# PRBonn/SHINE_mapping

Measured on AMD Instinct MI355X. Metric: trained SDF samples/sec (fwd+bwd), higher is better.
Workload: dtype f32; 1 GPU; maicity (BASELINE config 2): MaiCity-like 100 m street map, batch mode, 262144 points/iter/GPU, 4-level octree, F=8, decoder 8-32-32-1, BCE, f32; 100 poses x 64 beams x 1800 azimuths; points_per_iter_per_gpu=262144, levels=4, pool_samples=65450694, feature_table_bytes=14510624, parallelism=dp1

## Files before the change

include/shine_hip.h:

```cpp
#ifndef SHINE_HIP_H_
#define SHINE_HIP_H_

#include <stddef.h>
#include <stdint.h>

#ifdef __cplusplus
extern "C" {
#endif

#define SHINE_MAX_LEVELS 8
#define SHINE_FEATURE_DIM 8
#define SHINE_HIDDEN_DIM 32
#define SHINE_MLP_PARAMS 1377

#define SHINE_OK 0
#define SHINE_E_INVALID (-1)
#define SHINE_E_HIP (-2)
#define SHINE_E_NOMEM (-3)
#define SHINE_E_STATE (-4)

typedef struct shine_tables shine_tables;

#define SHINE_SURF_PARTS 64
typedef struct shine_next_draw {
  int64_t pool_size, n;
  uint64_t seed;
  uint64_t* stream_state;
  int32_t* idx_out;
  const uint32_t* surf_bits;
  int64_t* surf_parts;
  void* workspace;
} shine_next_draw;

typedef struct shine_draw_rider {
  int64_t pool_size, n;
  uint64_t seed;
  uint64_t* state;
  int32_t parity;
  double* block_sum[2];
  int32_t* idx_out;
  const uint32_t* surf_bits;
  int64_t* surf_parts[2];
  float* zero_ptr;
  int64_t zero_bytes;
} shine_draw_rider;
int shine_draw_rider_prime(const shine_draw_rider* r, uint64_t first_stream_id, void* stream);

typedef struct shine_reg_rider {
  const float* last[SHINE_MAX_LEVELS];
  const float* imp[SHINE_MAX_LEVELS];
  uint32_t* stamp[SHINE_MAX_LEVELS];
  uint32_t epoch;
  float* acc;
} shine_reg_rider;

typedef struct shine_step_config {
  int32_t n_levels;
  int32_t max_level;
  int32_t poly_int_on;
  int32_t reduction_sum;
  int32_t eikonal_on;
  int32_t decoder_grad_on;
  int32_t sorted_input;
  int32_t kernel_variant;
  float sigma;
  float weight_e;
  double inv_n;
  int64_t n_global;
  int32_t sort_origin[3];
  int32_t sort_bits[3];
  int32_t loss_weight_on;
  int64_t* adam_state;
  float adam_beta1, adam_beta2;
  double* zero_f64;
  int32_t n_surf_parts;
  const shine_next_draw* next_draw;
  int32_t defer_reduce;
// ... 259 lines not shown
```

shine_mapping_amd/_lib.py:

```python
import ctypes as C
import os

_HERE = os.path.dirname(os.path.abspath(__file__))
LIB_PATH = os.path.join(_HERE, "lib", "libshine_hip.so")
CHECK_LIB_PATH = os.path.join(_HERE, "lib", "libshine_check.so")

MAX_LEVELS = 8
FEATURE_DIM = 8
HIDDEN_DIM = 32
MLP_PARAMS = 1377


class NextDraw(C.Structure):
    _fields_ = [("pool_size", C.c_int64), ("n", C.c_int64), ("seed", C.c_uint64), ("stream_state", C.c_void_p),
                ("idx_out", C.c_void_p), ("surf_bits", C.c_void_p), ("surf_parts", C.c_void_p), ("workspace", C.c_void_p)]


class RegRider(C.Structure):

    _fields_ = [("last", C.c_void_p * 8), ("imp", C.c_void_p * 8), ("stamp", C.c_void_p * 8), ("epoch", C.c_uint32),
                ("acc", C.c_void_p)]


class DrawRider(C.Structure):

    _fields_ = [("pool_size", C.c_int64), ("n", C.c_int64), ("seed", C.c_uint64), ("state", C.c_void_p), ("parity", C.c_int32),
                ("block_sum", C.c_void_p * 2), ("idx_out", C.c_void_p), ("surf_bits", C.c_void_p), ("surf_parts", C.c_void_p * 2),
                ("zero_ptr", C.c_void_p), ("zero_bytes", C.c_int64)]


class StepConfig(C.Structure):

    _fields_ = [
        ("n_levels", C.c_int32),
        ("max_level", C.c_int32),
        ("poly_int_on", C.c_int32),
        ("reduction_sum", C.c_int32),
        ("eikonal_on", C.c_int32),
        ("decoder_grad_on", C.c_int32),
        ("sorted_input", C.c_int32),
        ("kernel_variant", C.c_int32),
        ("sigma", C.c_float),
        ("weight_e", C.c_float),
        ("inv_n", C.c_double),
        ("n_global", C.c_int64),
        ("sort_origin", C.c_int32 * 3),
        ("sort_bits", C.c_int32 * 3),
        ("loss_weight_on", C.c_int32),
        ("adam_state", C.c_void_p),
        ("adam_beta1", C.c_float),
        ("adam_beta2", C.c_float),
        ("zero_f64", C.c_void_p),
        ("n_surf_parts", C.c_int32),
        ("next_draw", C.POINTER(NextDraw)),
        ("defer_reduce", C.c_int32),
        ("reg_rider", C.POINTER(RegRider)),
        ("draw_rider", C.POINTER(DrawRider)),
    ]


_P = C.c_void_p
# ... 248 lines not shown
```

shine_mapping_amd/csrc/shine_graph.hip:

```cpp
#include <cstdlib>
#include <vector>

#include "shine_finish_args.hpp"
#include "shine_tile16.hpp"

struct shine_iter_graph {
  int unroll = 0;
  hipGraph_t graph = nullptr;
  hipGraphExec_t exec = nullptr;
  std::vector<hipGraphNode_t> step_nodes, fin_nodes;
  shine::StepLaunch step = {};
  shine::FinLaunch fin = {};
  bool have_step = false, have_fin = false, dirty = false;
  const void* built_step_fn = nullptr;
  const void* built_fin_fn = nullptr;
  long long commits = 0, builds = 0;
  hipEvent_t last_replay = nullptr;
  bool replayed = false;
  float* image = nullptr;
};

namespace shine {

static void graph_drop(shine_iter_graph* g) {
  if (g->exec) (void)hipGraphExecDestroy(g->exec);
  if (g->graph) (void)hipGraphDestroy(g->graph);
  g->exec = nullptr;
  g->graph = nullptr;
  g->step_nodes.clear();
  g->fin_nodes.clear();
}

static hipKernelNodeParams step_params(shine_iter_graph* g, void** kp) {
  hipKernelNodeParams p = {};
  kp[0] = &g->step.a;
  p.func = const_cast<void*>(g->step.fn);
  p.gridDim = g->step.grid;
  p.blockDim = g->step.block;
  p.sharedMemBytes = 0;
  p.kernelParams = kp;
  p.extra = nullptr;
  return p;
}

static hipKernelNodeParams fin_params(shine_iter_graph* g, void** kp) {
  hipKernelNodeParams p = {};
  kp[0] = &g->fin.a;
  kp[1] = &g->fin.fb;
  kp[2] = &g->fin.db;
  p.func = const_cast<void*>(g->fin.fn);
  p.gridDim = g->fin.grid;
  p.blockDim = g->fin.block;
  p.sharedMemBytes = 0;
  p.kernelParams = kp;
  p.extra = nullptr;
  return p;
}

static int graph_build(shine_iter_graph* g) {
  graph_drop(g);
  SHINE_HIP_CHECK(hipGraphCreate(&g->graph, 0));
  void* skp[1];
  void* fkp[3];
  hipKernelNodeParams sp = step_params(g, skp), fp = fin_params(g, fkp);
  hipGraphNode_t prev = nullptr;
  for (int u = 0; u < g->unroll; ++u) {
    hipGraphNode_t sn = nullptr, fn = nullptr;
    SHINE_HIP_CHECK(hipGraphAddKernelNode(&sn, g->graph, prev ? &prev : nullptr, prev ? 1 : 0, &sp));
    SHINE_HIP_CHECK(hipGraphAddKernelNode(&fn, g->graph, &sn, 1, &fp));
    g->step_nodes.push_back(sn);
    g->fin_nodes.push_back(fn);
    prev = fn;
  }
  SHINE_HIP_CHECK(hipGraphInstantiate(&g->exec, g->graph, nullptr, nullptr, 0));
  g->built_step_fn = g->step.fn;
  g->built_fin_fn = g->fin.fn;
  ++g->builds;
  return SHINE_OK;
}

}

using namespace shine;

extern "C" int shine_iter_graph_create(int32_t unroll, shine_iter_graph** out) {
  if (!out || unroll < 1 || unroll > 256) return set_error(SHINE_E_INVALID, "shine_iter_graph_create: 1 <= unroll <= 256");
  shine_iter_graph* g = new (std::nothrow) shine_iter_graph();
  if (!g) return set_error(SHINE_E_NOMEM, "shine_iter_graph_create: out of host memory");
  g->unroll = unroll;
  *out = g;
  return SHINE_OK;
}

extern "C" int shine_iter_graph_destroy(shine_iter_graph* g) {
  if (!g) return SHINE_OK;
// ... 43 lines not shown
                                           const int64_t* n_surf, double* loss_parts, const float* const* feats_last,
                                           const float* const* importance, unsigned char* const* touched,
                                           const int32_t* grad_on, float lambda_forget, double* reg_out, int32_t n_tensors,
                                           float* const* params, float* const* grads, float* const* exp_avg,
                                           float* const* exp_avg_sq, const int64_t* numel, const float* lr_dev,
                                           const int32_t* lr_index, const float* weight_decay, float beta1, float beta2,
                                           float eps, const int64_t* step_state, const shine_next_draw* next_draw,
                                           int32_t active_rows) {
  if (!g) return set_error(SHINE_E_INVALID, "shine_iter_graph_set_finish: null graph");
  FinLaunch fl;
  int rc = prepare_finish(&fl, cfg, n, workspace, n_surf, loss_parts, feats_last, importance, touched, grad_on, lambda_forget,
                          reg_out, n_tensors, params, grads, exp_avg, exp_avg_sq, numel, lr_dev, lr_index, weight_decay, beta1,
                          beta2, eps, step_state, next_draw, active_rows);
  if (rc != SHINE_OK) return rc;
  g->fin = fl;
  g->have_fin = true;
  g->dirty = true;
  return SHINE_OK;
}

extern "C" int shine_iter_graph_commit(shine_iter_graph* g) {
  if (!g || !g->have_step || !g->have_fin)
    return set_error(SHINE_E_STATE, "shine_iter_graph_commit: set_step and set_finish first");
  if (g->fin.a.partials != g->step.a.partials || g->fin.a.nblocks != g->step.blocks)
    return set_error(SHINE_E_INVALID, "shine_iter_graph_commit: the tail must consume the step's workspace (same buffer, same batch size)");
  g->fin.a.op_image = g->step.a.op_image ? g->image : nullptr;
  ++g->commits;
  g->dirty = false;
  if (g->replayed) {
    SHINE_HIP_CHECK(hipEventSynchronize(g->last_replay));
    g->replayed = false;
  }
  if (g->exec && g->built_step_fn == g->step.fn && g->built_fin_fn == g->fin.fn) {
    void* skp[1];
    void* fkp[3];
    hipKernelNodeParams sp = step_params(g, skp), fp = fin_params(g, fkp);
    bool ok = true;
    for (int u = 0; u < g->unroll && ok; ++u) {
      ok = hipGraphExecKernelNodeSetParams(g->exec, g->step_nodes[u], &sp) == hipSuccess &&
           hipGraphExecKernelNodeSetParams(g->exec, g->fin_nodes[u], &fp) == hipSuccess;
    }
    if (ok) return SHINE_OK;
    (void)hipGetLastError();
  }
  return graph_build(g);
}

extern "C" int shine_iter_graph_launch(shine_iter_graph* g, int32_t replays, void* stream) {
  if (!g || !g->exec || g->dirty) return set_error(SHINE_E_STATE, "shine_iter_graph_launch: commit first");
  if (replays < 1) return SHINE_OK;
  if (!g->last_replay) SHINE_HIP_CHECK(hipEventCreateWithFlags(&g->last_replay, hipEventDisableTiming));
  if (g->step.a.op_image) {
    const int rc = launch_operand_image(g->step.a, g->image, (hipStream_t)stream);
    if (rc != SHINE_OK) return rc;
  }
  for (int r = 0; r < replays; ++r) SHINE_HIP_CHECK(hipGraphLaunch(g->exec, (hipStream_t)stream));
  SHINE_HIP_CHECK(hipEventRecord(g->last_replay, (hipStream_t)stream));
  g->replayed = true;
  return SHINE_OK;
}

extern "C" int shine_iter_graph_stats(const shine_iter_graph* g, int64_t* commits, int64_t* builds) {
  if (!g) return set_error(SHINE_E_INVALID, "shine_iter_graph_stats: null graph");
  if (commits) *commits = g->commits;
  if (builds) *builds = g->builds;
  return SHINE_OK;
}
// ... 1 lines not shown
```

shine_mapping_amd/csrc/shine_step_common.hpp:

```cpp
#pragma once
#include "shine_internal.hpp"

namespace shine {

constexpr int LCAP = 4;

constexpr int PART_TRASH = SHINE_MLP_PARAMS;
constexpr int PART_FLOATS = PART_TRASH + SHINE_MAX_LEVELS * 8;
constexpr int PART_LOSS = 1444;
constexpr int PART_STRIDE = 1456;

struct V1Level {
  const unsigned long long* keys;
  const int4* vals;
  const float* feat;
  float* grad;
  unsigned int shift, mask;
  float res;
  int pad;
};

struct V1Args {
  V1Level lv[LCAP];
  long long rows[LCAP];
// ... 58 lines not shown
  const int cx = (c >> 2) & 1, cy = (c >> 1) & 1, cz = c & 1;
  const float px = cx ? X.t : 1.0f - X.t, py = cy ? Y.t : 1.0f - Y.t, pz = cz ? Z.t : 1.0f - Z.t;
  const float gx = cx ? X.dt : -X.dt, gy = cy ? Y.dt : -Y.dt, gz = cz ? Z.dt : -Z.dt;
  out[0] = gx * py * pz;
  out[1] = px * gy * pz;
  out[2] = px * py * gz;
}

typedef float f32x2_t __attribute__((ext_vector_type(2)));
__device__ __forceinline__ void corner_dw_pair(const Axis& X, const Axis& Y, const Axis& Z, int cp, f32x2_t out[3]) {
  const int cx = (cp >> 1) & 1, cy = cp & 1;
  const float px = cx ? X.t : 1.0f - X.t, py = cy ? Y.t : 1.0f - Y.t;
  const float gx = cx ? X.dt : -X.dt, gy = cy ? Y.dt : -Y.dt;
  const f32x2_t pz = {1.0f - Z.t, Z.t}, gz = {-Z.dt, Z.dt};
  const float a = gx * py, b = px * gy, c = px * py;
  out[0] = (f32x2_t){a, a} * pz;
  out[1] = (f32x2_t){b, b} * pz;
  out[2] = (f32x2_t){c, c} * gz;
}

__device__ __forceinline__ Axis axis_weight_rt(bool poly, float x, float res) {
  return poly ? axis_weight<true>(x, res, res * 0.5f) : axis_weight<false>(x, res, res * 0.5f);
}

struct V2Geometry {
  long long waves, chunk, blocks, tiles;
  int wg_waves;
};
V2Geometry v3_geometry(long long n, int ablate = 0);
long long v3_lds_bytes(int wg_waves);

extern long long* g_prof_buffer;

struct StepLaunch {
  const void* fn;
  dim3 grid, block;
  int blocks;
  bool mark_pass;
  V1Args a;
};
int prepare_step_v3(StepLaunch* out, const shine_tables* t, const shine_step_config* cfg, const float* coord,
                    const float* sdf_label, const float* weight, const int32_t* perm, const int32_t* slots,
                    const int64_t* n_surf, int64_t n, const float* const* feats, const int64_t* rows, const float* const* mlp,
                    float* pred_out, float* grad_x_out, float* const* grad_feats, float* const* grad_mlp, double* loss_parts,
                    unsigned char* const* touched, void* workspace, size_t workspace_bytes);

struct Pass1Args {
  double* block_sum;
  long long n1;
  unsigned long long seed;
  unsigned long long* stream_dev;
  long long* surf_parts;
  int nblocks;
};
struct DrawRiderArgs {
  const double* bs_next;
  double* bs_after;
  unsigned long long* state;
  int parity;
  int nblocks;
  long long n, pool;
  unsigned long long seed;
  int* idx;
  const unsigned int* surf_bits;
  long long* parts_this;
  long long* parts_next;
  float4* zero_ptr;
  long long zero_n16;
};
__global__ void k_reduce_partials(V1Args a, int nblocks, Pass1Args p1, DrawRiderArgs dr);
int fill_pass1_args(Pass1Args* p1, const shine_step_config* cfg);
int fill_draw_rider_args(DrawRiderArgs* dr, const shine_step_config* cfg);
__global__ void k_mark_touched(V1Args a);
int launch_operand_image(const V1Args& a, float* image, hipStream_t st);

inline int fill_step_args(V1Args* a, const shine_tables* t, const shine_step_config* cfg, const float* coord,
                          const float* sdf_label, const float* weight, const int32_t* perm, const int32_t* slots,
                          const int64_t* n_surf, int64_t n, const float* const* feats, const int64_t* rows,
                          const float* const* mlp, float* pred_out, float* grad_x_out, float* const* grad_feats,
                          float* const* grad_mlp, double* loss_parts, unsigned char* const* touched) {
  const bool rec_pool = cfg->sorted_input == 3;
  if (n < 0 || !feats || !rows || !mlp || !grad_feats || (n > 0 && (!coord || (!sdf_label && !rec_pool))))
    return set_error(SHINE_E_INVALID, "shine_train_step: null argument");
  if (rec_pool && (reinterpret_cast<uintptr_t>(coord) & 15))
    return set_error(SHINE_E_INVALID, "shine_train_step: a record pool must be 16-byte aligned");
  if (cfg->n_levels > LCAP) return set_error(SHINE_E_INVALID, "shine_train_step: the MFMA kernels handle up to 4 featured levels");
  const bool weight_inside = rec_pool && cfg->n_levels < 4;
  if (cfg->eikonal_on && ((!weight && !weight_inside) || !n_surf))
    return set_error(SHINE_E_INVALID, "shine_train_step: eikonal needs weight and n_surf");
  if (cfg->loss_weight_on && !weight && !weight_inside)
    return set_error(SHINE_E_INVALID, "shine_train_step: loss_weight_on needs weight");
  LevelSet ls = {};
  int rc = make_level_set(t, cfg, feats, rows, grad_feats, &ls);
  if (rc != SHINE_OK) return rc;
  for (int s = 0; s < cfg->n_levels; ++s) {
    if (!feats[s]) return set_error(SHINE_E_INVALID, "shine_train_step: null feature level");
    if (ls.lv[s].rows >= (1ll << 29)) return set_error(SHINE_E_INVALID, "shine_train_step: level exceeds 2^29 rows");
    a->lv[s].keys = ls.lv[s].keys;
    a->lv[s].vals = ls.lv[s].vals;
    a->lv[s].feat = ls.lv[s].feat;
    a->lv[s].grad = ls.lv[s].grad;
    a->lv[s].shift = ls.lv[s].shift;
    a->lv[s].mask = ls.lv[s].mask;
    a->lv[s].res = ls.lv[s].res;
    a->rows[s] = ls.lv[s].rows;
// ... 44 lines not shown
```

shine_mapping_amd/csrc/shine_step_support.hip:

```cpp
#include "shine_sampler_dev.hpp"
#include "shine_tile16.hpp"

namespace shine {

__global__ __launch_bounds__(256) void k_operand_image(V1Args a, float* image) {
  OperandRegs<256> R;
  decoder_operands_issue<256>(a, R, (int)threadIdx.x);
  decoder_operands_store<256>(R, image, image + V3_OPTOTAL, (int)threadIdx.x);
}

int launch_operand_image(const V1Args& a, float* image, hipStream_t st) {
  hipLaunchKernelGGL(k_operand_image, dim3(1), dim3(256), 0, st, a, image);
  SHINE_HIP_CHECK(hipGetLastError());
  return SHINE_OK;
}

__global__ __launch_bounds__(256) void k_mark_touched(V1Args a) {
  const long long i = (long long)blockIdx.x * 256 + threadIdx.x;
  if (i >= a.n) return;
  const int L = a.n_levels;
  float x0 = 0.f, x1 = 0.f, x2 = 0.f;
  const long long p = a.perm ? (long long)a.perm[i] : i;
  const long long si = a.pool_mode ? p : i;
  if (!a.slots && a.pool_mode != 2) {
    x0 = a.coord[3 * p];
    x1 = a.coord[3 * p + 1];
    x2 = a.coord[3 * p + 2];
  }
  for (int s = 0; s < L; ++s) {
    if (!a.touched[s]) continue;
    int sl;
    if (a.pool_mode == 2) {
      sl = reinterpret_cast<const int*>(a.coord)[8 * p + (L == 4 ? 4 : 5) + s];
    } else if (a.slots) {
      sl = a.slots[si * L + s];
    } else {
      LevelDev Lv = {};
      Lv.keys = a.lv[s].keys;
      Lv.shift = a.lv[s].shift;
      Lv.mask = a.lv[s].mask;
      Lv.res = a.lv[s].res;
      sl = level_slot(Lv, x0, x1, x2);
    }
    if (sl < 0) continue;
    int ids[8];
    corner_ids(a.lv[s].vals, (unsigned int)sl, ids);
    unsigned char* t = a.touched[s];
    for (int c = 0; c < 8; ++c) t[ids[c]] = 1;
  }
}

__device__ __forceinline__ void draw_rider_block(const DrawRiderArgs& dr, int rb) {
  __shared__ double s_red[4][4];
  __shared__ double s_wave_pre[4][4];
  __shared__ int s_cnt[4][4];
  const int qb = (dr.nblocks + 3) / 4;
  const int q = threadIdx.x >> 8, t256 = threadIdx.x & 255, w = t256 >> 6, lane = threadIdx.x & 63;
  const unsigned long long sid = dr.state[dr.parity];
  for (long long z = (long long)rb * 1024 + threadIdx.x; z < dr.zero_n16; z += (long long)2 * qb * 1024)
    dr.zero_ptr[z] = make_float4(0.f, 0.f, 0.f, 0.f);
  if (rb < qb) {
    const unsigned long long stream = sid + 2ull;
    const int vb = rb * 4 + q;
    if (rb == 0 && threadIdx.x == 0) dr.state[1 - dr.parity] = sid + 1ull;
    if (rb == 0 && dr.parts_this && threadIdx.x < SURF_PARTS) dr.parts_this[threadIdx.x] = 0;
    const long long k0 = (long long)vb * SB + t256 * 4;
    double v = 0.0;
#pragma unroll
    for (int j = 0; j < 4; ++j)
      if (vb < dr.nblocks && k0 + j < dr.n + 1) v += exp1v(dr.seed, stream, (unsigned long long)(k0 + j));
    v = wave_sum_d(v);
    if (lane == 0) s_red[q][w] = v;
    __syncthreads();
    if (t256 == 0 && vb < dr.nblocks) dr.bs_after[vb] = s_red[q][0] + s_red[q][1] + s_red[q][2] + s_red[q][3];
    return;
  }
  const unsigned long long stream = sid + 1ull;
  const int vb = (rb - qb) * 4 + q;
  const bool on = vb < dr.nblocks;
  double before = 0.0, total = 0.0;
  for (int b = t256; b < dr.nblocks; b += 256) {
    const double v = dr.bs_next[b];
    total += v;
    if (b < vb) before += v;
  }
  before = wave_sum_d(before);
  if (lane == 0) s_red[q][w] = before;
  __syncthreads();
  before = s_red[q][0] + s_red[q][1] + s_red[q][2] + s_red[q][3];
  __syncthreads();
  total = wave_sum_d(total);
  if (lane == 0) s_red[q][w] = total;
  __syncthreads();
  total = s_red[q][0] + s_red[q][1] + s_red[q][2] + s_red[q][3];
  __syncthreads();
  const long long k0 = (long long)vb * SB + t256 * 4;
  double e[4], run = 0.0;
#pragma unroll
  for (int j = 0; j < 4; ++j) {
    e[j] = (on && k0 + j <= dr.n) ? exp1v(dr.seed, stream, (unsigned long long)(k0 + j)) : 0.0;
    run += e[j];
  }
  double inc = run;
#pragma unroll
  for (int o = 1; o < 64; o <<= 1) {
    const double up = __shfl_up(inc, o, 64);
    if (lane >= o) inc += up;
  }
  if (lane == 63) s_wave_pre[q][w] = inc;
  __syncthreads();
  double wpre = 0.0;
  for (int ww = 0; ww < w; ++ww) wpre += s_wave_pre[q][ww];
  double sacc = before + wpre + (inc - run);
  int surf = 0;
#pragma unroll
  for (int j = 0; j < 4; ++j) {
    sacc += e[j];
    if (on && k0 + j < dr.n) {
      long long v = (long long)((sacc / total) * (double)dr.pool);
      v = v < 0 ? 0 : (v >= dr.pool ? dr.pool - 1 : v);
      dr.idx[k0 + j] = (int)v;
      if (dr.parts_next) surf += (int)((dr.surf_bits[v >> 5] >> (v & 31)) & 1u);
    }
  }
  if (dr.parts_next) {
#pragma unroll
    for (int o = 32; o > 0; o >>= 1) surf += __shfl_xor(surf, o, 64);
    if (lane == 0) s_cnt[q][w] = surf;
    __syncthreads();
    if (t256 == 0 && on)
      __hip_atomic_fetch_add(dr.parts_next + (vb & (SURF_PARTS - 1)), (long long)(s_cnt[q][0] + s_cnt[q][1] + s_cnt[q][2] + s_cnt[q][3]),
                             __ATOMIC_RELAXED, __HIP_MEMORY_SCOPE_AGENT);
  }
}

__global__ __launch_bounds__(1024) void k_reduce_partials(V1Args a, int nblocks, Pass1Args p1, DrawRiderArgs dr) {
  __shared__ float s_red[16][64];
  __shared__ double s_dred[16][3];
  constexpr int RB = (PART_FLOATS + 63) / 64;
  if ((int)blockIdx.x >= RB && dr.nblocks > 0) {
    draw_rider_block(dr, (int)blockIdx.x - RB);
    return;
  }
  if ((int)blockIdx.x >= RB) {
    __shared__ double s_p1[16];
    const unsigned long long stream = p1.stream_dev[0];
    const int vb = ((int)blockIdx.x - RB) * 4 + (int)(threadIdx.x >> 8), t256 = threadIdx.x & 255;
    if (vb == 0 && t256 == 0) p1.stream_dev[2] = stream + 1ull;
    if (vb == 0 && p1.surf_parts && t256 < SURF_PARTS) p1.surf_parts[t256] = 0;
    const long long k0 = (long long)vb * SB + t256 * 4;
    double v = 0.0;
#pragma unroll
    for (int j = 0; j < 4; ++j)
      if (vb < p1.nblocks && k0 + j < p1.n1) v += exp1v(p1.seed, stream, (unsigned long long)(k0 + j));
    v = wave_sum_d(v);
    if ((threadIdx.x & 63) == 0) s_p1[threadIdx.x >> 6] = v;
    __syncthreads();
    if (t256 == 0 && vb < p1.nblocks) {
      const int w = (int)(threadIdx.x >> 6);
      p1.block_sum[vb] = s_p1[w] + s_p1[w + 1] + s_p1[w + 2] + s_p1[w + 3];
    }
    return;
  }
  __shared__ long long s_ns;
  const int lane = threadIdx.x & 63, part = threadIdx.x >> 6;
  const int idx = blockIdx.x * 64 + lane;
  const int L = a.n_levels;
  float* dst = nullptr;
  if (part == 0 && idx < PART_FLOATS) {
    if (idx < SHINE_MLP_PARAMS) {
      if (a.decoder_grad_on) {
        if (idx < MLP_B1) dst = a.grad_mlp[0] + idx;
        else if (idx < MLP_W2) dst = a.grad_mlp[1] + (idx - MLP_B1);
        else if (idx < MLP_B2) dst = a.grad_mlp[2] + (idx - MLP_W2);
// ... 76 lines not shown
  }
  if (blockIdx.x == 1 && threadIdx.x < L * F) {
    const int sl = threadIdx.x / F, q = threadIdx.x % F;
    if (a.feat_rw[sl]) a.feat_rw[sl][a.rows[sl] * F + q] = 0.f;
  }
  if (blockIdx.x == RB - 1) {
    if (threadIdx.x == 0 && a.adam_state) adam_advance(a.adam_state, a.adam_b1, a.adam_b2);
    if (threadIdx.x == 64 && a.zero_f64) *a.zero_f64 = 0.0;
  }
}

__global__ void k_selftest_mfma16(const float* A, const float* B, float* D) {
  const int lane = threadIdx.x;
  f32x4 c = zero4();
  c = mfma16(A[(lane & 15) * 4 + (lane >> 4)], B[(lane >> 4) * 16 + (lane & 15)], c);
#pragma unroll
  for (int r = 0; r < 4; ++r) D[(4 * (lane >> 4) + r) * 16 + (lane & 15)] = c[r];
}

long long* g_prof_buffer = nullptr;

int fill_draw_rider_args(DrawRiderArgs* dr, const shine_step_config* cfg) {
  *dr = DrawRiderArgs{};
  const shine_draw_rider* r = cfg->draw_rider;
  if (!r) return SHINE_OK;
  if (cfg->next_draw || cfg->defer_reduce)
    return set_error(SHINE_E_INVALID, "shine_train_step: draw_rider excludes next_draw and defer_reduce");
  const long long nb = (r->n + 1 + SB - 1) / SB;
  if (r->n < 1 || nb > 0x3fffff || r->pool_size < 1 || r->pool_size > 0x7fffffffll || !r->state || !r->idx_out ||
      !r->block_sum[0] || !r->block_sum[1] || (r->parity != 0 && r->parity != 1) ||
      (r->surf_bits && (!r->surf_parts[0] || !r->surf_parts[1])))
    return set_error(SHINE_E_INVALID, "shine_train_step: draw_rider wants n >= 1, a device state, both block-sum buffers, idx_out, "
                                      "parity 0 / 1 and (with surf_bits) both surf_parts");
  if (r->zero_ptr && (((size_t)r->zero_ptr | (size_t)r->zero_bytes) & 15))
    return set_error(SHINE_E_INVALID, "shine_train_step: draw_rider's zero buffer must be 16-byte aligned and sized");
  dr->bs_next = r->block_sum[1 - r->parity];
  dr->bs_after = r->block_sum[r->parity];
  dr->state = reinterpret_cast<unsigned long long*>(r->state);
  dr->parity = r->parity;
  dr->nblocks = (int)nb;
  dr->n = r->n;
  dr->pool = r->pool_size;
  dr->seed = r->seed;
  dr->idx = r->idx_out;
  dr->surf_bits = r->surf_bits;
  dr->parts_this = r->surf_bits ? reinterpret_cast<long long*>(r->surf_parts[r->parity]) : nullptr;
  dr->parts_next = r->surf_bits ? reinterpret_cast<long long*>(r->surf_parts[1 - r->parity]) : nullptr;
  dr->zero_ptr = reinterpret_cast<float4*>(r->zero_ptr);
  dr->zero_n16 = r->zero_ptr ? r->zero_bytes / 16 : 0;
  return SHINE_OK;
}

int fill_pass1_args(Pass1Args* p1, const shine_step_config* cfg) {
  *p1 = Pass1Args{};
  const shine_next_draw* d = cfg->next_draw;
  if (!d) return SHINE_OK;
  const long long nb = (d->n + 1 + SB - 1) / SB;
  if (d->n < 1 || !d->stream_state || !d->workspace || nb > 0x3fffff)
    return set_error(SHINE_E_INVALID, "shine_train_step: next_draw wants n >= 1, a device stream state and the draw's workspace");
  p1->block_sum = reinterpret_cast<double*>(d->workspace);
  p1->n1 = d->n + 1;
  p1->seed = d->seed;
  p1->stream_dev = reinterpret_cast<unsigned long long*>(d->stream_state);
  p1->surf_parts = reinterpret_cast<long long*>(d->surf_parts);
  p1->nblocks = (int)nb;
  return SHINE_OK;
}

}

using namespace shine;

extern "C" void shine_debug_set_profile_buffer(int64_t* p) { g_prof_buffer = reinterpret_cast<long long*>(p); }

extern "C" int shine_selftest_mfma16(const float* a, const float* b, float* d, void* stream) {
  if (!a || !b || !d) return set_error(SHINE_E_INVALID, "shine_selftest_mfma16: null argument");
  hipLaunchKernelGGL(k_selftest_mfma16, dim3(1), dim3(64), 0, (hipStream_t)stream, a, b, d);
  SHINE_HIP_CHECK(hipGetLastError());
  return SHINE_OK;
}

extern "C" size_t shine_train_step_workspace_bytes(const shine_step_config* cfg, int64_t n) {
// ... 53 lines not shown
```

shine_mapping_amd/csrc/shine_step_v3.hip:

```cpp
#include "shine_step_body.hpp"

namespace shine {

template <int L, int WAVES, bool EIK, bool PROF, bool EXT = false, bool MARK = false, bool FAR = false>
__global__ __launch_bounds__(WAVES * 64, WAVES == V3_BIG ? V3_BIG / 4 : 2) void k_step_v3(V1Args a) {
  __shared__ StepShared<WAVES, FAR> sm;
  step_body<L, WAVES, EIK, PROF, EXT, MARK, false, FAR>(a, sm, (int)blockIdx.x, (int)gridDim.x);
}

__global__ void k_selftest_permlane(const float* x, const float* y, float* o32, float* o16) {
  const int lane = threadIdx.x;
  o32[lane] = xsum32(x[lane], y[lane]);
  o16[lane] = xsum16(x[lane], y[lane]);
}

V2Geometry v3_geometry(long long n, int ablate) {
  V2Geometry g;
  long long tiles = (n + V3_TP - 1) / V3_TP;
  if (tiles < 1) tiles = 1;
  g.tiles = tiles;
  g.wg_waves = tiles < 2048 ? 4 : V3_BIG;
  const long long max_waves = 256 * V3_BIG;
  const long long waves = tiles < max_waves ? tiles : max_waves;
  g.blocks = (waves + g.wg_waves - 1) / g.wg_waves;
  if (tiles <= 512 && (ablate & 128)) g.blocks = tiles;
  g.waves = g.blocks * g.wg_waves;
  g.chunk = 0;
  return g;
}

long long v3_lds_bytes(int wg_waves) {
  return (long long)sizeof(float) * (V3_OPTOTAL + 100 + (long long)wg_waves * V3_WAVE_FLOATS) +
         4 * sizeof(double);
}

template <int L, bool EIK, bool EXT, bool MARK>
static const void* step_fn_l(int wg_waves, bool prof, bool far) {
#if SHINE_V3_PROFBUILD
  if (prof && !EXT && !MARK) {
    if constexpr (L >= 3)
// ... 11 lines not shown
static const void* step_fn(int levels, int wg_waves, bool prof, bool far = false) {
  switch (levels) {
    case 1: return step_fn_l<1, EIK, EXT, MARK>(wg_waves, prof, far);
    case 2: return step_fn_l<2, EIK, EXT, MARK>(wg_waves, prof, far);
    case 3: return step_fn_l<3, EIK, EXT, MARK>(wg_waves, prof, far);
    default: return step_fn_l<4, EIK, EXT, MARK>(wg_waves, prof, far);
  }
}

constexpr long long FAR_TABLE_BYTES = 256ll << 20;
static bool far_regime(const shine_step_config* cfg, const int64_t* rows) {
  const int v = cfg->kernel_variant & 0xff;
  if (v == 6) return false;
  long long bytes = 0;
  for (int s = 0; s < cfg->n_levels; ++s) {
    if (rows[s] + 1 >= (1ll << V3_ROW_BITS)) return false;
    bytes += (rows[s] + 1) * (long long)(F * sizeof(float));
  }
  return v == 5 || bytes > FAR_TABLE_BYTES;
}

int prepare_step_v3(StepLaunch* out, const shine_tables* t, const shine_step_config* cfg, const float* coord,
                    const float* sdf_label, const float* weight, const int32_t* perm, const int32_t* slots,
                    const int64_t* n_surf, int64_t n, const float* const* feats, const int64_t* rows, const float* const* mlp,
                    float* pred_out, float* grad_x_out, float* const* grad_feats, float* const* grad_mlp, double* loss_parts,
                    unsigned char* const* touched, void* workspace, size_t workspace_bytes) {
  if (!slots && cfg->sorted_input != 3)
    return set_error(SHINE_E_INVALID, "shine_train_step_v3: needs a planned batch (slots)");
  if (cfg->sorted_input == 2)
    return set_error(SHINE_E_INVALID, "shine_train_step_v3: a pool batch is drawn from a RECORD pool (sorted_input 3: one 32-byte "
                                      "record per sample); the array form (2) is the importance sweep's");
  V1Args& a = out->a;
  a = V1Args{};
  int rc = fill_step_args(&a, t, cfg, coord, sdf_label, weight, perm, slots, n_surf, n, feats, rows, mlp, pred_out,
                          grad_x_out, grad_feats, grad_mlp, loss_parts, touched);
  if (rc != SHINE_OK) return rc;
  out->fn = nullptr;
  if (n == 0) return SHINE_OK;
  V2Geometry g = v3_geometry(n, a.ablate);
  if (a.ablate & 64) {
    g.blocks = 1;
    g.wg_waves = 4;
    g.waves = 4;
  }
  a.tiles = g.tiles;
  a.waves_total = g.waves;
  a.prof = g_prof_buffer;
  const size_t need = (size_t)g.blocks * PART_STRIDE * sizeof(float);
  if (!workspace || workspace_bytes < need)
    return set_error(SHINE_E_INVALID, "shine_train_step_v3: workspace too small (shine_train_step_workspace_bytes)");
  a.partials = (float*)workspace;
  bool mark_in_kernel = touched && !a.prof;
  for (int s = 0; s < cfg->n_levels; ++s) mark_in_kernel = mark_in_kernel && a.lv[s].grad != nullptr;
  out->mark_pass = touched && !mark_in_kernel;
  const bool prof = a.prof != nullptr;
  const bool far = far_regime(cfg, rows);
  if (mark_in_kernel)
    out->fn = cfg->eikonal_on ? step_fn<true, false, true>(cfg->n_levels, g.wg_waves, prof, far)
                              : step_fn<false, false, true>(cfg->n_levels, g.wg_waves, prof, far);
  else
    out->fn = cfg->eikonal_on ? step_fn<true, false, false>(cfg->n_levels, g.wg_waves, prof, far)
                              : step_fn<false, false, false>(cfg->n_levels, g.wg_waves, prof, far);
  out->grid = dim3((unsigned)g.blocks);
  out->block = dim3((unsigned)(g.wg_waves * 64));
  out->blocks = (int)g.blocks;
  return SHINE_OK;
}

}

using namespace shine;

extern "C" int shine_selftest_permlane(const float* x, const float* y, float* o32, float* o16, void* stream) {
  if (!x || !y || !o32 || !o16) return set_error(SHINE_E_INVALID, "shine_selftest_permlane: null argument");
  hipLaunchKernelGGL(k_selftest_permlane, dim3(1), dim3(64), 0, (hipStream_t)stream, x, y, o32, o16);
  SHINE_HIP_CHECK(hipGetLastError());
  return SHINE_OK;
}

extern "C" int shine_train_step_regime(const shine_step_config* cfg, const int64_t* rows, int64_t n, int32_t* far_out) {
  if (!cfg || !rows || !far_out) return set_error(SHINE_E_INVALID, "shine_train_step_regime: null argument");
  if (cfg->n_levels < 1 || cfg->n_levels > LCAP) return set_error(SHINE_E_INVALID, "shine_train_step_regime: 1..4 featured levels");
  *far_out = far_regime(cfg, rows) && cfg->n_levels >= 3 && v3_geometry(n > 0 ? n : 1).wg_waves == V3_BIG ? 1 : 0;
  return SHINE_OK;
}

extern "C" int shine_train_step_v3(const shine_tables* t, const shine_step_config* cfg, const float* coord,
                                   const float* sdf_label, const float* weight, const int32_t* perm,
                                   const int32_t* slots, const int64_t* n_surf, int64_t n, const float* const* feats,
                                   const int64_t* rows, const float* const* mlp, float* pred_out, float* grad_x_out,
                                   float* const* grad_feats, float* const* grad_mlp, double* loss_parts,
                                   unsigned char* const* touched, void* workspace, size_t workspace_bytes,
                                   void* stream) {
  StepLaunch sl;
  int rc = prepare_step_v3(&sl, t, cfg, coord, sdf_label, weight, perm, slots, n_surf, n, feats, rows, mlp, pred_out,
                           grad_x_out, grad_feats, grad_mlp, loss_parts, touched, workspace, workspace_bytes);
  if (rc != SHINE_OK) return rc;
  if (!sl.fn) return SHINE_OK;
  hipStream_t st = (hipStream_t)stream;
  V1Args& a = sl.a;
  if (sl.mark_pass) {
    hipLaunchKernelGGL(k_mark_touched, dim3((unsigned)((n + 255) / 256)), dim3(256), 0, st, a);
    SHINE_HIP_CHECK(hipGetLastError());
  }
  void* params[] = {&a};
  SHINE_HIP_CHECK(hipLaunchKernel(sl.fn, sl.grid, sl.block, params, 0, st));
  if (!(a.ablate & 32) && !a.defer_reduce) {
    Pass1Args p1;
    rc = fill_pass1_args(&p1, cfg);
    if (rc != SHINE_OK) return rc;
    DrawRiderArgs dr;
    rc = fill_draw_rider_args(&dr, cfg);
    if (rc != SHINE_OK) return rc;
    hipLaunchKernelGGL(k_reduce_partials,
                       dim3((unsigned)((PART_FLOATS + 63) / 64 + (p1.nblocks + 3) / 4 + 2 * ((dr.nblocks + 3) / 4))), dim3(1024), 0,
                       st, a, sl.blocks, p1, dr);
    SHINE_HIP_CHECK(hipGetLastError());
  }
  return SHINE_OK;
}

extern "C" int shine_interp_sdf_backward(const shine_tables* t, const shine_step_config* cfg, const float* coord,
                                         const int32_t* perm, const int32_t* slots, const float* grad_pred,
                                         const float* grad_g, int64_t n,
                                         const float* const* feats, const int64_t* rows, const float* const* mlp,
                                         float* const* grad_feats, float* const* grad_mlp, void* workspace,
                                         size_t workspace_bytes, void* stream) {
  if (!cfg || !perm || !slots || !grad_pred)
    return set_error(SHINE_E_INVALID, "shine_interp_sdf_backward: needs a planned batch (perm, slots) and grad_pred");
  if (cfg->eikonal_on || cfg->loss_weight_on || cfg->sorted_input == 2)
    return set_error(SHINE_E_INVALID, "shine_interp_sdf_backward: a plain planned batch, no loss options (the loss is the caller's: "
                                      "its eikonal part arrives as grad_g)");
  V1Args a = {};
  int rc = fill_step_args(&a, t, cfg, coord, coord, nullptr, perm, slots, nullptr, n, feats, rows, mlp, nullptr, nullptr,
                          grad_feats, grad_mlp, nullptr, nullptr);
  if (rc != SHINE_OK) return rc;
  if (n == 0) return SHINE_OK;
  a.ext_delta = grad_pred;
  a.ext_q = grad_g;
  a.inv_n = 1.0f;
  V2Geometry g = v3_geometry(n, a.ablate);
  if (a.ablate & 64) {
    g.blocks = 1;
    g.wg_waves = 4;
    g.waves = 4;
  }
  a.tiles = g.tiles;
  a.waves_total = g.waves;
  const size_t need = (size_t)g.blocks * PART_STRIDE * sizeof(float);
  if (!workspace || workspace_bytes < need)
    return set_error(SHINE_E_INVALID, "shine_interp_sdf_backward: workspace too small (shine_train_step_workspace_bytes)");
  a.partials = (float*)workspace;
  hipStream_t st = (hipStream_t)stream;
  void* params[] = {&a};
  const void* fn = grad_g ? step_fn<true, true, false>(cfg->n_levels, g.wg_waves, false)
                          : step_fn<false, true, false>(cfg->n_levels, g.wg_waves, false);
  SHINE_HIP_CHECK(hipLaunchKernel(fn, dim3((unsigned)g.blocks), dim3((unsigned)(g.wg_waves * 64)), params, 0, st));
  hipLaunchKernelGGL(k_reduce_partials, dim3((PART_FLOATS + 63) / 64), dim3(1024), 0, st, a, (int)g.blocks, Pass1Args{},
                     DrawRiderArgs{});
  SHINE_HIP_CHECK(hipGetLastError());
  return SHINE_OK;
}
```

shine_mapping_amd/sampler.py:

```python
import ctypes as C

import torch

from . import _lib
from .dp import plan_batch


def canonical_order(perm, slots):
    change = torch.ones(perm.numel(), dtype=torch.bool, device=perm.device)
    change[1:] = (slots[1:] != slots[:-1]).any(dim=1)
    key = (torch.cumsum(change, 0) << 32) + perm.long()
    return torch.argsort(key)


SURF_PARTS = 64

def importance_chunks(perm, n, bs, down_rate=1):
    import math

    n, bs, down_rate = int(n), int(bs), int(down_rate)
    n_chunks = math.ceil(n / (bs * down_rate))
    lib = _lib.lib()
    perm = perm.to(torch.int32).contiguous()
    idx = torch.empty(n, dtype=torch.int32, device=perm.device)
    begin = (C.c_int64 * (n_chunks + 1))()
    need = C.c_size_t()
    _lib.check(lib.shine_importance_chunks(None, n, bs, down_rate, None, None, n_chunks, None, C.byref(need), None),
               "shine_importance_chunks")
    ws = torch.empty(need.value, dtype=torch.uint8, device=perm.device)
    _lib.check(lib.shine_importance_chunks(perm.data_ptr(), n, bs, down_rate, idx.data_ptr(), begin, n_chunks, ws.data_ptr(),
                                           C.byref(need), _lib.current_stream_handle()), "shine_importance_chunks")
    largest = max((begin[c + 1] - begin[c] for c in range(n_chunks)), default=0)
    return idx, begin, n_chunks, largest


class DrawChain:

    def __init__(self, pool, n, idx, buckets=None, surf=False):
        dev = pool.device
        n = int(n)
        if not (idx.is_cuda and idx.dtype == torch.int32 and idx.is_contiguous() and idx.numel() == n):
            raise ValueError("DrawChain: idx must be a contiguous CUDA int32 tensor of n entries")
        self.pool, self.n, self.idx = pool, n, idx
        nb = (n + 1 + 1023) // 1024
        self.state = torch.zeros(2, dtype=torch.int64, device=dev)
        self.block_sum = (torch.zeros(nb, dtype=torch.float64, device=dev), torch.zeros(nb, dtype=torch.float64, device=dev))
        self.surf_parts = (pool.surf_parts_buffer(), pool.surf_parts_buffer()) if surf else (None, None)
        self.buckets = buckets
        self.parity = 0
        self.rider = []
        for p in (0, 1):
            r = _lib.DrawRider()
            r.pool_size, r.n, r.seed = pool.size, n, pool.seed
            r.state, r.parity = self.state.data_ptr(), p
            r.block_sum[0], r.block_sum[1] = self.block_sum[0].data_ptr(), self.block_sum[1].data_ptr()
            r.idx_out = idx.data_ptr()
            if surf:
                r.surf_bits = pool.surf_bits().data_ptr()
                r.surf_parts[0], r.surf_parts[1] = self.surf_parts[0].data_ptr(), self.surf_parts[1].data_ptr()
            if buckets is not None:
                z = buckets[1 - p]
                if not (z.is_cuda and z.is_contiguous() and z.data_ptr() % 16 == 0 and (z.numel() * z.element_size()) % 16 == 0):
                    raise ValueError("DrawChain: the gradient buckets must be contiguous, 16-byte aligned and sized")
                r.zero_ptr, r.zero_bytes = z.data_ptr(), z.numel() * z.element_size()
            self.rider.append(r)

    def prime(self, first_stream_id=None):
        if first_stream_id is None:
            self.pool._chains = getattr(self.pool, "_chains", 0) + 1
            first_stream_id = (self.pool._chains << 40) + int(self.pool.draws)
        sid = int(first_stream_id)
        _lib.check(_lib.lib().shine_draw_rider_prime(C.byref(self.rider[0]), sid, _lib.current_stream_handle()),
                   "shine_draw_rider_prime")
        self.first_stream_id = sid
        self.parity = 0
        return self


class SortedPool:
    def __init__(self, octree, coord, sdf_label, weight, seed=42, canonical=False):
        self.octree = octree
        self.canonical = bool(canonical)
        self.seed = int(seed)
        self.draws = 0
        self._ws = {}
        self._stream_state = None
        self._rider_for = None
        self.rebuild(coord, sdf_label, weight)

# ... 154 lines not shown
```

Baseline: 3.168 billion samples/s.

## Run next-iteration sample draw as trailing workgroups of the step kernel

Moves the draw-rider work (block sums, inverse-CDF index generation, surface counts, gradient bucket zeroing) out of the reduce kernel and into extra workgroups appended to the step kernel grid. The new indices go into a separate idx_next buffer, and the reduce kernel then only copies idx_next into idx with vectorized int4 stores and clears the surf parts. The aim is to overlap sampling with the fwd+bwd step and shorten the serialized tail kernel. In exchange it adds an extra index buffer, a copy pass, and workgroups that compete with the step for CUs.

```diff
diff --git a/include/shine_hip.h b/include/shine_hip.h
--- a/include/shine_hip.h
+++ b/include/shine_hip.h
@@ -43,6 +43,7 @@
   int64_t* surf_parts[2];
   float* zero_ptr;
   int64_t zero_bytes;
+  int32_t* idx_next;
 } shine_draw_rider;
 int shine_draw_rider_prime(const shine_draw_rider* r, uint64_t first_stream_id, void* stream);
 
diff --git a/shine_mapping_amd/_lib.py b/shine_mapping_amd/_lib.py
--- a/shine_mapping_amd/_lib.py
+++ b/shine_mapping_amd/_lib.py
@@ -26,7 +26,7 @@
 
     _fields_ = [("pool_size", C.c_int64), ("n", C.c_int64), ("seed", C.c_uint64), ("state", C.c_void_p), ("parity", C.c_int32),
                 ("block_sum", C.c_void_p * 2), ("idx_out", C.c_void_p), ("surf_bits", C.c_void_p), ("surf_parts", C.c_void_p * 2),
-                ("zero_ptr", C.c_void_p), ("zero_bytes", C.c_int64)]
+                ("zero_ptr", C.c_void_p), ("zero_bytes", C.c_int64), ("idx_next", C.c_void_p)]
 
 
 class StepConfig(C.Structure):
diff --git a/shine_mapping_amd/csrc/shine_draw_rider.hpp b/shine_mapping_amd/csrc/shine_draw_rider.hpp
--- /dev/null
+++ b/shine_mapping_amd/csrc/shine_draw_rider.hpp
@@ -0,0 +1,94 @@
+#pragma once
+#include "shine_sampler_dev.hpp"
+#include "shine_step_common.hpp"
+
+namespace shine {
+
+template <int Q>
+__device__ __forceinline__ void draw_rider_block(const DrawRiderArgs& dr, int rb, int* idx, bool clear_this) {
+  __shared__ double s_red[Q][4];
+  __shared__ double s_wave_pre[Q][4];
+  __shared__ int s_cnt[Q][4];
+  const int qb = (dr.nblocks + Q - 1) / Q;
+  const int q = threadIdx.x >> 8, t256 = threadIdx.x & 255, w = t256 >> 6, lane = threadIdx.x & 63;
+  const unsigned long long sid = dr.state[dr.parity];
+  for (long long z = (long long)rb * (Q * 256) + threadIdx.x; z < dr.zero_n16; z += (long long)2 * qb * (Q * 256))
+    dr.zero_ptr[z] = make_float4(0.f, 0.f, 0.f, 0.f);
+  if (rb < qb) {
+    const unsigned long long stream = sid + 2ull;
+    const int vb = rb * Q + q;
+    if (rb == 0 && threadIdx.x == 0) dr.state[1 - dr.parity] = sid + 1ull;
+    if (clear_this && rb == 0 && dr.parts_this && threadIdx.x < SURF_PARTS) dr.parts_this[threadIdx.x] = 0;
+    const long long k0 = (long long)vb * SB + t256 * 4;
+    double v = 0.0;
+#pragma unroll
+    for (int j = 0; j < 4; ++j)
+      if (vb < dr.nblocks && k0 + j < dr.n + 1) v += exp1v(dr.seed, stream, (unsigned long long)(k0 + j));
+    v = wave_sum_d(v);
+    if (lane == 0) s_red[q][w] = v;
+    __syncthreads();
+    if (t256 == 0 && vb < dr.nblocks) dr.bs_after[vb] = s_red[q][0] + s_red[q][1] + s_red[q][2] + s_red[q][3];
+    return;
+  }
+  const unsigned long long stream = sid + 1ull;
+  const int vb = (rb - qb) * Q + q;
+  const bool on = vb < dr.nblocks;
+  double before = 0.0, total = 0.0;
+  for (int b = t256; b < dr.nblocks; b += 256) {
+    const double v = dr.bs_next[b];
+    total += v;
+    if (b < vb) before += v;
+  }
+  before = wave_sum_d(before);
+  if (lane == 0) s_red[q][w] = before;
+  __syncthreads();
+  before = s_red[q][0] + s_red[q][1] + s_red[q][2] + s_red[q][3];
+  __syncthreads();
+  total = wave_sum_d(total);
+  if (lane == 0) s_red[q][w] = total;
+  __syncthreads();
+  total = s_red[q][0] + s_red[q][1] + s_red[q][2] + s_red[q][3];
+  __syncthreads();
+  const long long k0 = (long long)vb * SB + t256 * 4;
+  double e[4], run = 0.0;
+#pragma unroll
+  for (int j = 0; j < 4; ++j) {
+    e[j] = (on && k0 + j <= dr.n) ? exp1v(dr.seed, stream, (unsigned long long)(k0 + j)) : 0.0;
+    run += e[j];
+  }
+  double inc = run;
+#pragma unroll
+  for (int o = 1; o < 64; o <<= 1) {
+    const double up = __shfl_up(inc, o, 64);
+    if (lane >= o) inc += up;
+  }
+  if (lane == 63) s_wave_pre[q][w] = inc;
+  __syncthreads();
+  double wpre = 0.0;
+  for (int ww = 0; ww < w; ++ww) wpre += s_wave_pre[q][ww];
+  double sacc = before + wpre + (inc - run);
+  int surf = 0;
+#pragma unroll
+  for (int j = 0; j < 4; ++j) {
+    sacc += e[j];
+    if (on && k0 + j < dr.n) {
+      long long v = (long long)((sacc / total) * (double)dr.pool);
+      v = v < 0 ? 0 : (v >= dr.pool ? dr.pool - 1 : v);
+      idx[k0 + j] = (int)v;
+      if (dr.parts_next) surf += (int)((dr.surf_bits[v >> 5] >> (v & 31)) & 1u);
+    }
+  }
+  if (dr.parts_next) {
+#pragma unroll
+    for (int o = 32; o > 0; o >>= 1) surf += __shfl_xor(surf, o, 64);
+    if (lane == 0) s_cnt[q][w] = surf;
+    __syncthreads();
+    if (t256 == 0 && on)
+      __hip_atomic_fetch_add(dr.parts_next + (vb & (SURF_PARTS - 1)), (long long)(s_cnt[q][0] + s_cnt[q][1] + s_cnt[q][2] + s_cnt[q][3]),
+                             __ATOMIC_RELAXED, __HIP_MEMORY_SCOPE_AGENT);
+  }
+}
+
+inline int draw_rider_workgroups(int nblocks, int q) { return 2 * ((nblocks + q - 1) / q); }
+
+}
diff --git a/shine_mapping_amd/csrc/shine_graph.hip b/shine_mapping_amd/csrc/shine_graph.hip
--- a/shine_mapping_amd/csrc/shine_graph.hip
+++ b/shine_mapping_amd/csrc/shine_graph.hip
@@ -34,6 +34,7 @@
 static hipKernelNodeParams step_params(shine_iter_graph* g, void** kp) {
   hipKernelNodeParams p = {};
   kp[0] = &g->step.a;
+  kp[1] = &g->step.dr;
   p.func = const_cast<void*>(g->step.fn);
   p.gridDim = g->step.grid;
   p.blockDim = g->step.block;
@@ -60,7 +61,7 @@
 static int graph_build(shine_iter_graph* g) {
   graph_drop(g);
   SHINE_HIP_CHECK(hipGraphCreate(&g->graph, 0));
-  void* skp[1];
+  void* skp[2];
   void* fkp[3];
   hipKernelNodeParams sp = step_params(g, skp), fp = fin_params(g, fkp);
   hipGraphNode_t prev = nullptr;
@@ -170,7 +171,7 @@
     g->replayed = false;
   }
   if (g->exec && g->built_step_fn == g->step.fn && g->built_fin_fn == g->fin.fn) {
-    void* skp[1];
+    void* skp[2];
     void* fkp[3];
     hipKernelNodeParams sp = step_params(g, skp), fp = fin_params(g, fkp);
     bool ok = true;
diff --git a/shine_mapping_amd/csrc/shine_step_common.hpp b/shine_mapping_amd/csrc/shine_step_common.hpp
--- a/shine_mapping_amd/csrc/shine_step_common.hpp
+++ b/shine_mapping_amd/csrc/shine_step_common.hpp
@@ -114,19 +114,6 @@
 
 extern long long* g_prof_buffer;
 
-struct StepLaunch {
-  const void* fn;
-  dim3 grid, block;
-  int blocks;
-  bool mark_pass;
-  V1Args a;
-};
-int prepare_step_v3(StepLaunch* out, const shine_tables* t, const shine_step_config* cfg, const float* coord,
-                    const float* sdf_label, const float* weight, const int32_t* perm, const int32_t* slots,
-                    const int64_t* n_surf, int64_t n, const float* const* feats, const int64_t* rows, const float* const* mlp,
-                    float* pred_out, float* grad_x_out, float* const* grad_feats, float* const* grad_mlp, double* loss_parts,
-                    unsigned char* const* touched, void* workspace, size_t workspace_bytes);
-
 struct Pass1Args {
   double* block_sum;
   long long n1;
@@ -149,10 +136,30 @@
   long long* parts_next;
   float4* zero_ptr;
   long long zero_n16;
-};
+  int* idx_next;
+  int on_tail;
+  int copy_vec;
+};
+
+struct StepLaunch {
+  const void* fn;
+  dim3 grid, block;
+  int blocks;
+  bool mark_pass;
+  bool tail_ok;
+  V1Args a;
+  DrawRiderArgs dr;
+};
+int prepare_step_v3(StepLaunch* out, const shine_tables* t, const shine_step_config* cfg, const float* coord,
+                    const float* sdf_label, const float* weight, const int32_t* perm, const int32_t* slots,
+                    const int64_t* n_surf, int64_t n, const float* const* feats, const int64_t* rows, const float* const* mlp,
+                    float* pred_out, float* grad_x_out, float* const* grad_feats, float* const* grad_mlp, double* loss_parts,
+                    unsigned char* const* touched, void* workspace, size_t workspace_bytes);
+
 __global__ void k_reduce_partials(V1Args a, int nblocks, Pass1Args p1, DrawRiderArgs dr);
 int fill_pass1_args(Pass1Args* p1, const shine_step_config* cfg);
 int fill_draw_rider_args(DrawRiderArgs* dr, const shine_step_config* cfg);
+constexpr int IDX_COPY_BLOCK = 4096;
 __global__ void k_mark_touched(V1Args a);
 int launch_operand_image(const V1Args& a, float* image, hipStream_t st);
 
diff --git a/shine_mapping_amd/csrc/shine_step_support.hip b/shine_mapping_amd/csrc/shine_step_support.hip
--- a/shine_mapping_amd/csrc/shine_step_support.hip
+++ b/shine_mapping_amd/csrc/shine_step_support.hip
@@ -1,4 +1,4 @@
-#include "shine_sampler_dev.hpp"
+#include "shine_draw_rider.hpp"
 #include "shine_tile16.hpp"
 
 namespace shine {
@@ -50,96 +50,25 @@
   }
 }
 
-__device__ __forceinline__ void draw_rider_block(const DrawRiderArgs& dr, int rb) {
-  __shared__ double s_red[4][4];
-  __shared__ double s_wave_pre[4][4];
-  __shared__ int s_cnt[4][4];
-  const int qb = (dr.nblocks + 3) / 4;
-  const int q = threadIdx.x >> 8, t256 = threadIdx.x & 255, w = t256 >> 6, lane = threadIdx.x & 63;
-  const unsigned long long sid = dr.state[dr.parity];
-  for (long long z = (long long)rb * 1024 + threadIdx.x; z < dr.zero_n16; z += (long long)2 * qb * 1024)
-    dr.zero_ptr[z] = make_float4(0.f, 0.f, 0.f, 0.f);
-  if (rb < qb) {
-    const unsigned long long stream = sid + 2ull;
-    const int vb = rb * 4 + q;
-    if (rb == 0 && threadIdx.x == 0) dr.state[1 - dr.parity] = sid + 1ull;
-    if (rb == 0 && dr.parts_this && threadIdx.x < SURF_PARTS) dr.parts_this[threadIdx.x] = 0;
-    const long long k0 = (long long)vb * SB + t256 * 4;
-    double v = 0.0;
-#pragma unroll
-    for (int j = 0; j < 4; ++j)
-      if (vb < dr.nblocks && k0 + j < dr.n + 1) v += exp1v(dr.seed, stream, (unsigned long long)(k0 + j));
-    v = wave_sum_d(v);
-    if (lane == 0) s_red[q][w] = v;
-    __syncthreads();
-    if (t256 == 0 && vb < dr.nblocks) dr.bs_after[vb] = s_red[q][0] + s_red[q][1] + s_red[q][2] + s_red[q][3];
-    return;
-  }
-  const unsigned long long stream = sid + 1ull;
-  const int vb = (rb - qb) * 4 + q;
-  const bool on = vb < dr.nblocks;
-  double before = 0.0, total = 0.0;
-  for (int b = t256; b < dr.nblocks; b += 256) {
-    const double v = dr.bs_next[b];
-    total += v;
-    if (b < vb) before += v;
-  }
-  before = wave_sum_d(before);
-  if (lane == 0) s_red[q][w] = before;
-  __syncthreads();
-  before = s_red[q][0] + s_red[q][1] + s_red[q][2] + s_red[q][3];
-  __syncthreads();
-  total = wave_sum_d(total);
-  if (lane == 0) s_red[q][w] = total;
-  __syncthreads();
-  total = s_red[q][0] + s_red[q][1] + s_red[q][2] + s_red[q][3];
-  __syncthreads();
-  const long long k0 = (long long)vb * SB + t256 * 4;
-  double e[4], run = 0.0;
-#pragma unroll
-  for (int j = 0; j < 4; ++j) {
-    e[j] = (on && k0 + j <= dr.n) ? exp1v(dr.seed, stream, (unsigned long long)(k0 + j)) : 0.0;
-    run += e[j];
-  }
-  double inc = run;
-#pragma unroll
-  for (int o = 1; o < 64; o <<= 1) {
-    const double up = __shfl_up(inc, o, 64);
-    if (lane >= o) inc += up;
-  }
-  if (lane == 63) s_wave_pre[q][w] = inc;
-  __syncthreads();
-  double wpre = 0.0;
-  for (int ww = 0; ww < w; ++ww) wpre += s_wave_pre[q][ww];
-  double sacc = before + wpre + (inc - run);
-  int surf = 0;
-#pragma unroll
-  for (int j = 0; j < 4; ++j) {
-    sacc += e[j];
-    if (on && k0 + j < dr.n) {
-      long long v = (long long)((sacc / total) * (double)dr.pool);
-      v = v < 0 ? 0 : (v >= dr.pool ? dr.pool - 1 : v);
-      dr.idx[k0 + j] = (int)v;
-      if (dr.parts_next) surf += (int)((dr.surf_bits[v >> 5] >> (v & 31)) & 1u);
-    }
-  }
-  if (dr.parts_next) {
-#pragma unroll
-    for (int o = 32; o > 0; o >>= 1) surf += __shfl_xor(surf, o, 64);
-    if (lane == 0) s_cnt[q][w] = surf;
-    __syncthreads();
-    if (t256 == 0 && on)
-      __hip_atomic_fetch_add(dr.parts_next + (vb & (SURF_PARTS - 1)), (long long)(s_cnt[q][0] + s_cnt[q][1] + s_cnt[q][2] + s_cnt[q][3]),
-                             __ATOMIC_RELAXED, __HIP_MEMORY_SCOPE_AGENT);
-  }
-}
-
 __global__ __launch_bounds__(1024) void k_reduce_partials(V1Args a, int nblocks, Pass1Args p1, DrawRiderArgs dr) {
   __shared__ float s_red[16][64];
   __shared__ double s_dred[16][3];
   constexpr int RB = (PART_FLOATS + 63) / 64;
+  if ((int)blockIdx.x >= RB && dr.nblocks > 0 && dr.on_tail) {
+    const int cb = (int)blockIdx.x - RB;
+    if (cb == 0 && dr.parts_this && threadIdx.x < SURF_PARTS) dr.parts_this[threadIdx.x] = 0;
+    const long long i4 = (long long)cb * IDX_COPY_BLOCK + 4 * (long long)threadIdx.x;
+    if (dr.copy_vec && i4 + 3 < dr.n) {
+      *reinterpret_cast<int4*>(dr.idx + i4) = *reinterpret_cast<const int4*>(dr.idx_next + i4);
+    } else {
+#pragma unroll
+      for (int j = 0; j < 4; ++j)
+        if (i4 + j < dr.n) dr.idx[i4 + j] = dr.idx_next[i4 + j];
+    }
+    return;
+  }
   if ((int)blockIdx.x >= RB && dr.nblocks > 0) {
-    draw_rider_block(dr, (int)blockIdx.x - RB);
+    draw_rider_block<4>(dr, (int)blockIdx.x - RB, dr.idx, true);
     return;
   }
   if ((int)blockIdx.x >= RB) {
@@ -282,6 +211,8 @@
       (r->surf_bits && (!r->surf_parts[0] || !r->surf_parts[1])))
     return set_error(SHINE_E_INVALID, "shine_train_step: draw_rider wants n >= 1, a device state, both block-sum buffers, idx_out, "
                                       "parity 0 / 1 and (with surf_bits) both surf_parts");
+  if (r->idx_next && r->idx_next == r->idx_out)
+    return set_error(SHINE_E_INVALID, "shine_train_step: draw_rider's idx_next must be a buffer of its own (the running step reads idx_out)");
   if (r->zero_ptr && (((size_t)r->zero_ptr | (size_t)r->zero_bytes) & 15))
     return set_error(SHINE_E_INVALID, "shine_train_step: draw_rider's zero buffer must be 16-byte aligned and sized");
   dr->bs_next = r->block_sum[1 - r->parity];
@@ -298,6 +229,8 @@
   dr->parts_next = r->surf_bits ? reinterpret_cast<long long*>(r->surf_parts[1 - r->parity]) : nullptr;
   dr->zero_ptr = reinterpret_cast<float4*>(r->zero_ptr);
   dr->zero_n16 = r->zero_ptr ? r->zero_bytes / 16 : 0;
+  dr->idx_next = r->idx_next;
+  dr->copy_vec = (((size_t)r->idx_out | (size_t)r->idx_next) & 15) == 0;
   return SHINE_OK;
 }
 
diff --git a/shine_mapping_amd/csrc/shine_step_v3.hip b/shine_mapping_amd/csrc/shine_step_v3.hip
--- a/shine_mapping_amd/csrc/shine_step_v3.hip
+++ b/shine_mapping_amd/csrc/shine_step_v3.hip
@@ -1,11 +1,22 @@
+#include "shine_draw_rider.hpp"
 #include "shine_step_body.hpp"
 
 namespace shine {
 
 template <int L, int WAVES, bool EIK, bool PROF, bool EXT = false, bool MARK = false, bool FAR = false>
-__global__ __launch_bounds__(WAVES * 64, WAVES == V3_BIG ? V3_BIG / 4 : 2) void k_step_v3(V1Args a) {
+__global__ __launch_bounds__(WAVES * 64, WAVES == V3_BIG ? V3_BIG / 4 : 2) void k_step_v3(V1Args a, DrawRiderArgs dr) {
   __shared__ StepShared<WAVES, FAR> sm;
-  step_body<L, WAVES, EIK, PROF, EXT, MARK, false, FAR>(a, sm, (int)blockIdx.x, (int)gridDim.x);
+  if constexpr (!PROF && !EXT) {
+    static_assert(WAVES % 4 == 0, "a trailing workgroup is WAVES / 4 sampler blocks of 256 threads");
+    const int step_blocks = (int)(a.waves_total / WAVES);
+    if ((int)blockIdx.x >= step_blocks) {
+      draw_rider_block<WAVES / 4>(dr, (int)blockIdx.x - step_blocks, dr.idx_next, false);
+      return;
+    }
+    step_body<L, WAVES, EIK, PROF, EXT, MARK, false, FAR>(a, sm, (int)blockIdx.x, step_blocks);
+  } else {
+    step_body<L, WAVES, EIK, PROF, EXT, MARK, false, FAR>(a, sm, (int)blockIdx.x, (int)gridDim.x);
+  }
 }
 
 __global__ void k_selftest_permlane(const float* x, const float* y, float* o32, float* o16) {
@@ -83,6 +94,8 @@
                                       "record per sample); the array form (2) is the importance sweep's");
   V1Args& a = out->a;
   a = V1Args{};
+  out->dr = DrawRiderArgs{};
+  out->tail_ok = false;
   int rc = fill_step_args(&a, t, cfg, coord, sdf_label, weight, perm, slots, n_surf, n, feats, rows, mlp, pred_out,
                           grad_x_out, grad_feats, grad_mlp, loss_parts, touched);
   if (rc != SHINE_OK) return rc;
@@ -112,6 +125,7 @@
   else
     out->fn = cfg->eikonal_on ? step_fn<true, false, false>(cfg->n_levels, g.wg_waves, prof, far)
                               : step_fn<false, false, false>(cfg->n_levels, g.wg_waves, prof, far);
+  out->tail_ok = !SHINE_V3_PROFBUILD || !prof;
   out->grid = dim3((unsigned)g.blocks);
   out->block = dim3((unsigned)(g.wg_waves * 64));
   out->blocks = (int)g.blocks;
@@ -154,18 +168,24 @@
     hipLaunchKernelGGL(k_mark_touched, dim3((unsigned)((n + 255) / 256)), dim3(256), 0, st, a);
     SHINE_HIP_CHECK(hipGetLastError());
   }
-  void* params[] = {&a};
+  const bool reduce = !(a.ablate & 32) && !a.defer_reduce;
+  DrawRiderArgs dr = {};
+  if (reduce) rc = fill_draw_rider_args(&dr, cfg);
+  if (rc != SHINE_OK) return rc;
+  if (dr.nblocks > 0 && dr.idx_next && sl.tail_ok) {
+    dr.on_tail = 1;
+    sl.dr = dr;
+    sl.grid.x += (unsigned)draw_rider_workgroups(dr.nblocks, (int)sl.block.x / 256);
+  }
+  void* params[] = {&a, &sl.dr};
   SHINE_HIP_CHECK(hipLaunchKernel(sl.fn, sl.grid, sl.block, params, 0, st));
-  if (!(a.ablate & 32) && !a.defer_reduce) {
+  if (reduce) {
     Pass1Args p1;
     rc = fill_pass1_args(&p1, cfg);
     if (rc != SHINE_OK) return rc;
-    DrawRiderArgs dr;
-    rc = fill_draw_rider_args(&dr, cfg);
-    if (rc != SHINE_OK) return rc;
-    hipLaunchKernelGGL(k_reduce_partials,
-                       dim3((unsigned)((PART_FLOATS + 63) / 64 + (p1.nblocks + 3) / 4 + 2 * ((dr.nblocks + 3) / 4))), dim3(1024), 0,
-                       st, a, sl.blocks, p1, dr);
+    const int rider_blocks = dr.on_tail ? (int)((dr.n + IDX_COPY_BLOCK - 1) / IDX_COPY_BLOCK) : draw_rider_workgroups(dr.nblocks, 4);
+    hipLaunchKernelGGL(k_reduce_partials, dim3((unsigned)((PART_FLOATS + 63) / 64 + (p1.nblocks + 3) / 4 + rider_blocks)),
+                       dim3(1024), 0, st, a, sl.blocks, p1, dr);
     SHINE_HIP_CHECK(hipGetLastError());
   }
   return SHINE_OK;
@@ -203,7 +223,8 @@
     return set_error(SHINE_E_INVALID, "shine_interp_sdf_backward: workspace too small (shine_train_step_workspace_bytes)");
   a.partials = (float*)workspace;
   hipStream_t st = (hipStream_t)stream;
-  void* params[] = {&a};
+  DrawRiderArgs no_rider = {};
+  void* params[] = {&a, &no_rider};
   const void* fn = grad_g ? step_fn<true, true, false>(cfg->n_levels, g.wg_waves, false)
                           : step_fn<false, true, false>(cfg->n_levels, g.wg_waves, false);
   SHINE_HIP_CHECK(hipLaunchKernel(fn, dim3((unsigned)g.blocks), dim3((unsigned)(g.wg_waves * 64)), params, 0, st));
diff --git a/shine_mapping_amd/sampler.py b/shine_mapping_amd/sampler.py
--- a/shine_mapping_amd/sampler.py
+++ b/shine_mapping_amd/sampler.py
@@ -47,6 +47,7 @@
         self.block_sum = (torch.zeros(nb, dtype=torch.float64, device=dev), torch.zeros(nb, dtype=torch.float64, device=dev))
         self.surf_parts = (pool.surf_parts_buffer(), pool.surf_parts_buffer()) if surf else (None, None)
         self.buckets = buckets
+        self.idx_next = torch.empty_like(idx)
         self.parity = 0
         self.rider = []
         for p in (0, 1):
@@ -55,6 +56,7 @@
             r.state, r.parity = self.state.data_ptr(), p
             r.block_sum[0], r.block_sum[1] = self.block_sum[0].data_ptr(), self.block_sum[1].data_ptr()
             r.idx_out = idx.data_ptr()
+            r.idx_next = self.idx_next.data_ptr()
             if surf:
                 r.surf_bits = pool.surf_bits().data_ptr()
                 r.surf_parts[0], r.surf_parts[1] = self.surf_parts[0].data_ptr(), self.surf_parts[1].data_ptr()
```

Result: faster. 3.258 billion samples/s (median of 6 runs) (+2.8%).
